# leejet/stable-diffusion.cpp

Hardware: AMD Instinct MI355X
Metric: denoise it/s (image-iterations/s: cond+uncond UNet forwards per image per step) (higher is better)
Workload: dtype f16; 1 GPU; sd15 UNet 512x512, cfg 7 (cond+uncond), f16 weights, batch 8/GPU, Euler-A step; global_batch=8, flash_attn=True, hip_graph=1, cfg_pair_in_one_graph=True, device_resident_sampler=True

## Files before the change

include/ggml-mi355x.h:

```cpp
#ifndef GGML_MI355X_H
#define GGML_MI355X_H

#include "ggml-abi.h"

#ifdef __cplusplus
extern "C" {
#endif

#define GGML_MI355X_API __attribute__((visibility("default")))

GGML_MI355X_API ggml_backend_reg_t ggml_backend_init(void);
GGML_MI355X_API int ggml_backend_score(void);
GGML_MI355X_API ggml_backend_reg_t ggml_backend_mi355x_reg(void);
GGML_MI355X_API int ggml_backend_mi355x_get_device_count(void);

struct ggml_backend_mi355x_stats {
    int64_t graphs_computed;
    int64_t plans_built;
    int64_t nodes_seen;
    int64_t kernels_planned;
    int64_t kernels_launched;
    int64_t fused_conv;
    int64_t fused_conv_bounced;
    int64_t fused_linear;
// ... 16 lines not shown
    int64_t fused_proj_tokens;
    int64_t gemm_attention;
    int64_t fused_q16;
    int64_t split_k_inlaunch;
    int64_t qgemm16_linears;
    int64_t fgemv_linears;
    int64_t fused_presilu;
    int64_t fused_sibling_linears;
    int64_t hoisted_kv_linears;
    int64_t window_convs;
    int64_t hoisted_emb_linears;
    int64_t fused_rows16;
    int64_t fused_joint_qkv;
    int64_t jit_images;
    int64_t fused_cat_rows16;
    int64_t fused_gn_stats;
    int64_t fused_ln_reduce;
    int64_t redirect_fallbacks;
    int64_t fused_concat_gn;
    int64_t fused_conv_scale;
    int64_t view_graphs;
    int64_t plans_evicted;
    int64_t hoisted_mod_linears;
    int64_t view_external_nodes;
    int64_t qinloop_linears;
    int64_t flash_out_alias;
    int64_t flash_slice_images;
    int64_t flash_short_launches;
    int64_t flash_qb2_launches;
    int64_t flash_mslot_launches;
    int64_t flash_generic_launches;
    int64_t fused_gn_epilogue;
    int64_t fused_tile_merge;
};
GGML_MI355X_API void ggml_backend_mi355x_get_stats(struct ggml_backend_mi355x_stats* out);
GGML_MI355X_API int ggml_backend_mi355x_resolve_enums(const char* (*op_name)(int), const char* (*unary_op_name)(int), const char* (*type_name)(int));
GGML_MI355X_API const char* ggml_backend_mi355x_enum_status(void);
GGML_MI355X_API void ggml_backend_mi355x_get_enum_maps(uint8_t* ops256, uint8_t* unary256);
struct ggml_backend_mi355x_kernel_timing {
    char kernel[96];
    int64_t launches;
    double total_ms;
    double total_flops;
    double total_bytes;
    int32_t bound;
    int32_t family;
};
GGML_MI355X_API void ggml_backend_mi355x_kernel_timing_enable(int enable);
GGML_MI355X_API void ggml_backend_mi355x_kernel_timing_enable_mask(uint32_t family_mask);
GGML_MI355X_API void ggml_backend_mi355x_get_kernel_timing(struct ggml_backend_mi355x_kernel_timing* out);
GGML_MI355X_API int ggml_backend_mi355x_get_kernel_timings(struct ggml_backend_mi355x_kernel_timing* out, int capacity);
GGML_MI355X_API void ggml_backend_mi355x_set_option(const char* key, int value);
struct ggml_backend_mi355x_calibration {
    float mfma_f16_tflops;
    float mfma_clock_mhz;
    float copy_tbs;
    float read_tbs;
    int compute_units;
};
GGML_MI355X_API int ggml_backend_mi355x_calibrate(struct ggml_backend_mi355x_calibration* out);
GGML_MI355X_API void* ggml_backend_mi355x_get_stream(ggml_backend_t backend);
GGML_MI355X_API bool ggml_backend_mi355x_step_cache_probe(ggml_backend_t backend, const float* x, float c_in, const float* prev_in, int64_t n, float* stats);
GGML_MI355X_API bool ggml_backend_mi355x_step_cache_record(ggml_backend_t backend, const float* in, const float* out, float* prev_in, float* prev_out, float* diff, int64_t per,
                                                           int k, int64_t nb, bool has_prev_out, float* stats);
GGML_MI355X_API bool ggml_backend_mi355x_step_cache_probe_rel(ggml_backend_t backend, const float* x, float c_in, const float* prev_in, int64_t n, float* stats);
GGML_MI355X_API bool ggml_backend_mi355x_spectrum_predict(ggml_backend_t backend, const float* ring, int64_t slot_stride, const int* order, int k, const float* weights, float w,
                                                          int64_t n, float* out);
GGML_MI355X_API bool ggml_backend_mi355x_spectrum_push(ggml_backend_t backend, const float* src, float* dst, int64_t n);
GGML_MI355X_API const char* ggml_backend_mi355x_hip_library(void);
GGML_MI355X_API int ggml_backend_mi355x_set_device(int hip_device);
GGML_MI355X_API int ggml_backend_mi355x_get_device(void);

#ifdef __cplusplus
}
#endif
#endif
```

stable-diffusion.cpp_amd/__init__.py:

```python
from __future__ import annotations

import ctypes as C
import os
from pathlib import Path

import numpy as np

PKG_DIR = Path(__file__).resolve().parent
ROOT = PKG_DIR.parent
LIB_DIR = PKG_DIR / "lib"
HOST_LIB = Path(os.environ.get("SDCPP_HOST_LIB", str(LIB_DIR / "libsdcpp-host.so")))
BACKEND_LIB = Path(os.environ.get("SDCPP_BACKEND_LIB", str(LIB_DIR / "libggml-mi355x.so")))

F32, F16, Q4_0, Q8_0, I32, BF16 = 0, 1, 2, 8, 26, 30
TYPE_SIZE = {F32: 4, F16: 2, BF16: 2, I32: 4}

SD15, SDXL, SD15_TINY, SDXL_TINY, SD35_LARGE, SD35_TINY, FLUX_DEV, FLUX_TINY, SD35_WIDE2, FLUX_WIDE1, SD3M_TINY, SD35_WIDE8, FLUX_WIDE8 = 0, 1, 2, 3, 4, 5, 6, 7, 8, 9, 10, 11, 12
PAIR_EXCHANGE_FN = C.CFUNCTYPE(C.c_bool, C.c_void_p, C.c_int64, C.c_void_p, C.c_void_p)
EVAL_CALLBACK_FN = C.CFUNCTYPE(C.c_bool, C.c_void_p, C.c_bool, C.c_void_p)
EULER, EULER_A, HEUN, DPM2, DPMPP2S_A, DPMPP2M, DPMPP2Mv2, IPNDM, IPNDM_V, LCM, DDIM_TRAILING = range(11)
TCD, RES_MULTISTEP, RES_2S, ER_SDE, EULER_CFG_PP, EULER_A_CFG_PP, EULER_GE, DPMPP2M_SDE, DPMPP2M_SDE_BT, LMS = range(11, 21)
SAMPLE_METHOD_DEFAULT = 21
SCHED_DISCRETE, SCHED_KARRAS, SCHED_EXPONENTIAL, SCHED_AYS, SCHED_GITS, SCHED_SGM_UNIFORM, SCHED_SIMPLE, SCHED_SMOOTHSTEP, SCHED_KL_OPTIMAL, SCHED_LCM = range(10)
SCHED_BONG_TANGENT, SCHED_FLUX, SCHED_BETA, SCHEDULER_DEFAULT = 10, 14, 15, 16
# ... 319 lines not shown
    L.sd_get_learned_condition.restype = C.c_bool
    L.sdm_set_backend_eval_callback.argtypes = [EVAL_CALLBACK_FN, C.c_void_p]
    L.sdm_set_backend_eval_callback.restype = None
    L.sdm_backend_graph_compute_with_eval_callback.argtypes = [C.c_void_p, C.c_void_p, EVAL_CALLBACK_FN, C.c_void_p]
    L.sdm_backend_graph_compute_with_eval_callback.restype = C.c_int
    _lib = L
    return L


_loaded_plugins: set[str] = set()


def load_backend(path: os.PathLike | str) -> None:
    p = str(Path(path).resolve())
    if p in _loaded_plugins:
        return
    if not lib().sd_load_backend(p.encode()):
        raise EngineError(f"failed to load backend plug-in {p}")
    _loaded_plugins.add(p)


def load_mi355x_backend() -> None:
    if not BACKEND_LIB.exists():
        raise EngineError(f"{BACKEND_LIB} missing — the HIP backend was not built")
    load_backend(BACKEND_LIB)
    names = devices()
    if not any(n.upper().startswith("MI355X") for n in names):
        raise EngineError(f"libggml-mi355x.so loaded but exposes no MI355X device (devices: {names}); is a gfx950 GPU visible?")


_BACKEND_STAT_FIELDS = ("graphs_computed plans_built nodes_seen kernels_planned kernels_launched fused_conv fused_conv_bounced fused_linear "
                        "fused_norm fused_geglu fused_attention generic_matmul swizzled_weight_bytes graph_replays fused_linear_geglu "
                        "split_k_gemms head_major_gemms fused_modulate fused_gate fused_gelu fused_rope fused_concat_heads qgemv_linears fused_chan_add fused_proj_tokens gemm_attention fused_q16 split_k_inlaunch qgemm16_linears fgemv_linears fused_presilu fused_sibling_linears hoisted_kv_linears window_convs hoisted_emb_linears fused_rows16 fused_joint_qkv jit_images fused_cat_rows16 fused_gn_stats fused_ln_reduce redirect_fallbacks fused_concat_gn fused_conv_scale view_graphs plans_evicted hoisted_mod_linears view_external_nodes qinloop_linears flash_out_alias flash_slice_images "
                        "flash_short_launches flash_qb2_launches flash_mslot_launches flash_generic_launches fused_gn_epilogue fused_tile_merge").split()


class BackendStats(C.Structure):
    _fields_ = [(n, C.c_int64) for n in _BACKEND_STAT_FIELDS]


_backend_cdll = None


def _backend() -> C.CDLL:
    global _backend_cdll
    if _backend_cdll is None:
        load_mi355x_backend()
        _backend_cdll = C.CDLL(str(BACKEND_LIB))
        _backend_cdll.ggml_backend_mi355x_get_stats.argtypes = [C.POINTER(BackendStats)]
        _backend_cdll.ggml_backend_mi355x_set_option.argtypes = [C.c_char_p, C.c_int]
    return _backend_cdll


def backend_stats() -> dict:
    st = BackendStats()
    _backend().ggml_backend_mi355x_get_stats(C.byref(st))
    return {n: int(getattr(st, n)) for n in _BACKEND_STAT_FIELDS}


class KernelTiming(C.Structure):
    _fields_ = [("kernel", C.c_char * 96), ("launches", C.c_int64), ("total_ms", C.c_double), ("total_flops", C.c_double),
                ("total_bytes", C.c_double), ("bound", C.c_int32), ("family", C.c_int32)]


KF_ALL = 0x3FFFF


# ... 722 lines not shown
```

stable-diffusion.cpp_amd/csrc/backend/backend.cpp:

```cpp
#include <hip/hip_runtime.h>

#include <atomic>
#include <cstdio>
#include <cstdlib>
#include <cstring>
#include <mutex>
#include <string>
#include <vector>

#include "ggml-abi.h"
#include "ggml-abi-check.h"
#include <dlfcn.h>
#include <link.h>

#include "ggml-mi355x.h"
#include "ktime.h"
#include "planner.h"
#include "kernels.h"

namespace mi355x {

#define HIP_OK(expr)                                                                                          \
    do {                                                                                                      \
        hipError_t _e = (expr);                                                                               \
// ... 364 lines not shown
    return (int)mi355x::g_devices.size();
}
GGML_MI355X_API void ggml_backend_mi355x_get_stats(struct ggml_backend_mi355x_stats* out) { mi355x::planner_get_stats(out); }
GGML_MI355X_API int ggml_backend_mi355x_calibrate(struct ggml_backend_mi355x_calibration* out) {
    mi355x::CalibrationResult r;
    if (!out || !mi355x::calibrate_device(nullptr, &r)) return -1;
    out->mfma_f16_tflops = r.mfma_f16_tflops;
    out->mfma_clock_mhz  = r.mfma_clock_mhz;
    out->copy_tbs        = r.copy_tbs;
    out->read_tbs        = r.read_tbs;
    out->compute_units   = r.compute_units;
    return 0;
}
GGML_MI355X_API int ggml_backend_mi355x_resolve_enums(const char* (*op_name)(int), const char* (*unary_op_name)(int), const char* (*type_name)(int)) {
    std::lock_guard<std::mutex> lk(mi355x::g_enum_mu);
    const bool was_ok = mi355x::g_enum_ok;
    const std::string was = mi355x::g_enum_status;
    const bool ok = mi355x::resolve_host_enums(op_name, unary_op_name, type_name, "ggml_backend_mi355x_resolve_enums");
    if (ok) {
        mi355x::g_enum_explicit = true;
    } else {
        mi355x::g_enum_ok     = was_ok;
        mi355x::g_enum_status = mi355x::g_enum_status + " [previous state kept: " + was + "]";
    }
    return ok ? 0 : -1;
}
GGML_MI355X_API const char* ggml_backend_mi355x_enum_status(void) {
    std::lock_guard<std::mutex> lk(mi355x::g_enum_mu);
    static thread_local std::string copy;
    copy = mi355x::g_enum_status;
    return copy.c_str();
}
GGML_MI355X_API void ggml_backend_mi355x_get_enum_maps(uint8_t* ops256, uint8_t* unary256) { mi355x::planner_get_op_maps(ops256, unary256); }
GGML_MI355X_API void ggml_backend_mi355x_set_option(const char* key, int value) {
    if (strcmp(key, "pinned_uploads") == 0) {
        mi355x::g_pinned_uploads.store(value);
        return;
    }
    mi355x::planner_set_option(key, value);
}
static void fill_timing(struct ggml_backend_mi355x_kernel_timing* o, const mi355x::KFamTiming& t, int family) {
    memset(o, 0, sizeof(*o));
    snprintf(o->kernel, sizeof(o->kernel), "%s", t.name);
    o->launches    = t.launches;
    o->total_ms    = t.total_ms;
    o->total_flops = t.total_flops;
    o->total_bytes = t.total_bytes;
    o->bound       = t.bound;
    o->family      = family;
}
GGML_MI355X_API void ggml_backend_mi355x_kernel_timing_enable(int enable) { mi355x::ktime_enable(enable ? 1u : 0u); }
GGML_MI355X_API void ggml_backend_mi355x_kernel_timing_enable_mask(uint32_t family_mask) { mi355x::ktime_enable(family_mask); }
GGML_MI355X_API void* ggml_backend_mi355x_get_stream(ggml_backend_t backend) {
    return backend ? (void*)((mi355x::BackendCtx*)backend->context)->stream : nullptr;
}
static float* step_cache_scratch(mi355x::BackendCtx* c) {
    if (!c->step_cache_partial && hipMalloc((void**)&c->step_cache_partial, mi355x::step_cache_partial_bytes()) != hipSuccess) {
        (void)hipGetLastError();
        c->step_cache_partial = nullptr;
    }
    return c->step_cache_partial;
}
GGML_MI355X_API bool ggml_backend_mi355x_step_cache_probe(ggml_backend_t backend, const float* x, float c_in, const float* prev_in, int64_t n, float* stats) {
    if (!backend || !x || !prev_in || !stats) return false;
    mi355x::BackendCtx* c = (mi355x::BackendCtx*)backend->context;
    if (hipSetDevice(c->dev->id) != hipSuccess) return false;
// ... 64 lines not shown
```

stable-diffusion.cpp_amd/csrc/backend/planner.cpp:

```cpp
#include "planner.h"

#include <atomic>
#include <cstddef>
#include <cstdio>
#include <cstdlib>
#include <cstring>
#include <functional>
#include <memory>
#include <mutex>
#include <string>
#include <algorithm>
#include <map>
#include <unordered_map>
#include <unordered_set>
#include <vector>

#include "kernels.h"
#include "ktime.h"

namespace mi355x {

static uint8_t g_opmap[256];
static uint8_t g_unmap[256];
static bool g_opmap_init = [] {
// ... 76 lines not shown
        err_len = sizeof(local);
    }
    static const char* const kOptionalOps[]   = {"CONV_2D"};
    static const char* const kOptionalUnary[] = {"EXP"};
    if (op_name && !build_map(op_name, kNeededOps, (int)(sizeof(kNeededOps) / sizeof(kNeededOps[0])), 200, GGML_OP_COUNT, ops, err, err_len, "op", kOptionalOps, 1)) return false;
    if (unary_name && !build_map(unary_name, kNeededUnary, (int)(sizeof(kNeededUnary) / sizeof(kNeededUnary[0])), 64, GGML_UNARY_OP_COUNT, un, err, err_len, "unary op", kOptionalUnary, 1))
        return false;
    if (type_name) {
        for (const NameNum& t : kNeededTypes) {
            const char* nm = type_name(t.num);
            if (!nm || strcmp(nm, t.name)) {
                snprintf(err, err_len, "host ggml_type %d is named '%s', this backend was written against '%s'", t.num, nm ? nm : "(null)", t.name);
                return false;
            }
        }
    }
    if (op_name) memcpy(g_opmap, ops, 256);
    if (unary_name) memcpy(g_unmap, un, 256);
    return true;
}
void planner_get_op_maps(uint8_t* ops256, uint8_t* unary256) {
    if (ops256) memcpy(ops256, g_opmap, 256);
    if (unary256) memcpy(unary256, g_unmap, 256);
}

namespace {

constexpr size_t N_STATS = sizeof(ggml_backend_mi355x_stats) / sizeof(int64_t);
static_assert(N_STATS * sizeof(int64_t) == sizeof(ggml_backend_mi355x_stats), "ggml_backend_mi355x_stats: int64_t fields only");
std::atomic<int64_t> g_stat_counters[N_STATS];
#define STAT(field) g_stat_counters[offsetof(ggml_backend_mi355x_stats, field) / sizeof(int64_t)]

struct Options {
    std::atomic<int> fusion{1}, mfma_gemm{1}, hip_graph{1}, flash_pattern{1}, fuse_modulate{1}, fuse_gate{1}, fuse_gelu{1}, fuse_rope{1}, fuse_concat_heads{1}, qgemv{1}, fuse_chan_add{1}, fuse_proj_tokens{1}, fuse_q16{1}, qgemm16{1}, fgemv{1}, fuse_siblings{1}, hoist_kv{1}, hoist_emb{1}, fuse_rows16{0}, fuse_cat_rows16{1}, fuse_joint_qkv{1}, jit_qimages{4096}, fuse_gn_stats{1}, fuse_ln_reduce{1}, relax_res_overlap{1}, fuse_split_gelu{1}, fuse_concat_gn{1}, fuse_gn_tokens{1}, fuse_linear_nchw{1}, fuse_conv_scale{1}, ignore_use_counts{0}, plan_cache_cap{512}, hoist_mod{1}, fuse_flash_slices{1}, fuse_act_pack{1}, fuse_gn_epilogue{1}, fuse_tile_merge{1};
} g_opt;

using Step = std::function<void(hipStream_t)>;

struct Plan {
    int n_nodes = 0;
    uint64_t check = 0;
    size_t arena_needed = 0;
    std::vector<Step> steps;
    hipGraphExec_t graph_exec = nullptr;
    bool graph_failed         = false;
    int64_t runs              = 0;
    uint64_t last_use         = 0;
};

struct SwzEntry {
    void* swz;
    size_t bytes;
    const void* src;
    size_t src_bytes;
};

std::mutex g_mu;
std::vector<Planner*> g_planners;

}

struct Planner {
    int device;
    std::mutex mu;
    uint64_t tick = 0;
    std::unordered_map<uint64_t, std::unique_ptr<Plan>> plans;
    std::unordered_map<uint64_t, SwzEntry> swz;
// ... 830 lines not shown
        return;
    }
    if (g_opt.fgemv && plain_epi && simple_rows && src_safe && emit_node == i && fgemv_supported((int)w->type, tokens, K) && aligned16(w->data)) {
        float* fdst       = (float*)gi.node(last)->data;
        const float* fx   = (const float*)xsrc->data;
        const int64_t fxs = (int64_t)x->nb[1] / 4;
        const void* wp    = w->data;
        const int wt      = (int)w->type;
        const bool silu   = xsrc != x;
        B.emit([=](hipStream_t st) { launch_fgemv(st, fdst, M, fx, fxs, tokens, wp, wt, K, M, ep, silu); });
        STAT(fgemv_linears)++;
        STAT(fused_linear)++;
        if (silu) STAT(fused_presilu)++;
        return;
    }
    if (xsrc != x) {
        float* ud       = (float*)x->data;
        const float* us = (const float*)xsrc->data;
        const int64_t un = ggml_abi_nelements(x);
        B.emit([=](hipStream_t st) { launch_unary(st, UN_SILU, ud, us, un); });
    }
    const bool useq  = g_opt.qgemm16 && hm_d == 0 && geglu_out < 0 && qgemm16_supported((int)w->type, tokens, K, M);
    const void* wraw = w->data;
    const int wt     = (int)w->type;
    const bool qin = !useq && geglu_out < 0 && hm_d == 0 && !B.hm_hoisting && nchw_add < 0 && (wt == 8 || wt == 2) &&
                     (int64_t)w->nb[1] == (int64_t)ggml_abi_row_size(w->type, K) && aligned16(w->data) && gemm16_qinloop_supported(wt, tokens, M, K, 1, 1);
    if (qin) {
        ep.qtype      = wt;
        ep.qrow_bytes = (int64_t)w->nb[1];
        STAT(qinloop_linears)++;
    }
    const bool jit = !useq && !qin && g_opt.jit_qimages > 0 && tokens >= g_opt.jit_qimages && geglu_out < 0 && hm_d == 0 && !B.hm_hoisting && wswz_q_supported((int)w->type, K) &&
                     (int64_t)w->nb[1] == (int64_t)ggml_abi_row_size(w->type, K) && aligned16(w->data);
    const int geglu_mode = geglu_out >= 0 ? gemm16_geglu_mode(tokens, M, K) : 0;
    const void* swz = useq ? nullptr : qin ? w->data : (jit ? B.P->jit_buffer(wswz_bytes(M, K), B.jit_seq[wswz_bytes(M, K)]++) : get_swz_linear(B.P, w, s, geglu_mode));
    if (jit && swz) {
        void* jb          = const_cast<void*>(swz);
        const void* wsrc  = w->data;
        const int wty     = (int)w->type;
        B.emit_at(emit_node, i, [=](hipStream_t st) { launch_wswz_q(st, jb, wsrc, wty, K, M); });
        STAT(jit_images)++;
    }
    float* dst      = (float*)gi.node(last)->data;
    const float* xp = (const float*)x->data;
    const int64_t xs = (int64_t)x->nb[1] / 4;
    const ggml_tensor* key = strip_reshape(x);
    auto it = B.packed.find(key);
    if (it == B.packed.end() || it->second.nhwc) {
        Packed pk{B.alloc((size_t)tokens * rup64(K) * 2), rup64(K), false};
        Planner* P = B.P;
        const size_t off = pk.off;
        const bool runs  = x->ne[2] > 1 && x->nb[2] != x->nb[1] * (size_t)x->ne[1];
        const int64_t pL = runs ? x->ne[1] : 0, pbs = runs ? (int64_t)x->nb[2] / 4 : 0;
        B.emit([=](hipStream_t st) { launch_pack_rows_f16(st, P->arena + off, xp, tokens, K, xs, pL, pbs); });
        it = B.packed.emplace(key, pk).first;
        if (it->second.nhwc) it->second = pk;
    }
    Planner* P       = B.P;
    size_t off       = it->second.off;
    const int64_t ld = it->second.ld;
    if (it->second.runL > 0) {
        const int64_t rL = it->second.runL, rS = it->second.runS;
        if (geglu_out >= 0 || hm_d > 0 || nchw_add >= 0) {
            const size_t goff = B.alloc((size_t)tokens * ld * 2), soff = off;
            const int64_t nrun = tokens / rL;
            B.emit([=](hipStream_t st) {
                for (int64_t r = 0; r < nrun; ++r)
                    (void)hipMemcpyAsync(P->arena + goff + (size_t)(r * rL * ld * 2), P->arena + soff + (size_t)(r * rS * ld * 2), (size_t)(rL * ld * 2), hipMemcpyDeviceToDevice, st);
            });
            off = goff;
        } else {
            ep.a_run_L = rL;
            ep.a_run_S = rS;
        }
    }
    if (nchw_add >= 0 && !useq && swz && ld == rup64(K) && geglu_out < 0 && gelu_out < 0 && !ep.gate && !redir) {
        float* ndst             = (float*)gi.node(nchw_add)->data;
        const int64_t HWt = nchw_HW, Nimg = nchw_N;
        const float* resp       = nchw_res;
        const Builder::Split sk = B.plan_split(tokens, M, rup64(K), true, true);
        const bool rec_want = g_opt.fuse_gn_epilogue && feeds_group_norm(gi, nchw_add);
        const bool rec_on  = sk.S <= 1 && rec_want && gemm16_conv_gn_rec_supported(HWt, Nimg, M, rup64(K), 1);
        const size_t rec_o = rec_on ? B.alloc((size_t)Nimg * (HWt / GN_REC_CHUNK) * M * sizeof(GnRec)) : 0;
        if (rec_on) B.gn_rec[gi.node(nchw_add)] = rec_o;
        B.emit_at(emit_node, i, [=](hipStream_t st) {
            Epilogue e2 = ep;
            e2.residual = resp;
            if (rec_on) e2.gn_rec = (GnRec*)(P->arena + rec_o);
            launch_gemm16_conv(st, ndst, P->arena + off, swz, HWt, 1, K, Nimg, M, 1, 1, 0, false, e2, sk.ws(P), sk.cnt(P), sk.S);
        });
        STAT(fused_linear)++;
        STAT(fused_proj_tokens)++;
        return;
    }
    if (nchw_add >= 0) {
        while (!chain.empty() && chain.back() != last) chain.pop_back();
    }
    if (geglu_out >= 0) {
        const size_t ooff  = B.alloc((size_t)tokens * (M / 2) * 2);
        const float* biasp = ep.bias;
        const Builder::Split sk = B.plan_split(tokens, M, K, false, false, true);
        B.emit([=](hipStream_t st) { launch_gemm16_linear_geglu(st, P->arena + ooff, P->arena + off, ld, swz, tokens, K, M, biasp, sk.ws(P), sk.cnt(P), sk.S, geglu_mode); });
        B.packed[gi.node(geglu_out)] = Packed{ooff, M / 2, false};
        STAT(fused_geglu)++;
        STAT(fused_linear_geglu)++;
    } else if (gelu_out >= 0) {
        const size_t ooff = B.alloc((size_t)tokens * M * 2);
        if (useq) {
            B.emit([=](hipStream_t st) { launch_qgemm16(st, nullptr, P->arena + ooff, M, P->arena + off, ld, tokens, wraw, wt, K, M, ep); });
            STAT(qgemm16_linears)++;
        } else {
            const Builder::Split sk = B.plan_split(tokens, M, K, false, false);
            B.emit([=](hipStream_t st) { launch_gemm16_linear(st, nullptr, P->arena + ooff, M, P->arena + off, ld, swz, tokens, K, M, M, ep, 0, 0, 0, sk.ws(P), sk.cnt(P), sk.S); });
        }
        B.packed[gi.node(gelu_out)] = Packed{ooff, M, false};
        STAT(fused_gelu)++;
    } else if (hm_d > 0) {
        void* hdst = gi.node(last)->data;
        STAT(head_major_gemms)++;
        const bool f16o = hm_f16;
        const int hd = hm_d, hH = hm_H, hL = hm_L;
        int qflash = -1, qview = -1;
        if (!f16o && g_opt.fuse_q16 && hd % 8 == 0) {
            const int c1 = gi.sole(last);
            const int c2 = (c1 >= 0 && xop(gi.node(c1)) == GGML_OP_RESHAPE) ? gi.sole(c1) : -1;
            if (c2 >= 0 && xop(gi.node(c2)) == GGML_OP_FLASH_ATTN_EXT && gi.node(c2)->src[0] == gi.node(c1) && !gi.node(c2)->src[3] && contig(gi.node(c1)) &&
                gi.node(c1)->ne[0] == hd && flash_attn_supported(hd, gi.node(c2)->src[2]->ne[0])) {
                qflash = c2;
                qview  = c1;
            }
        }
        const bool groupable = B.hm_grouping && !ep.residual && !ep.gate && !ep.gelu && !ep.chan_add;
        if (qflash >= 0) {
            const size_t qoff        = B.alloc((size_t)tokens * M * 2);
            B.q16[gi.node(qview)]    = qoff;
// ... 82 lines not shown
                    if (b2 < 0 || b2 % 4 != 0 || col2 + v2->ne[0] > c0) others_ok = false;
                }
                if (!others_ok) continue;
                split_on  = true;
                split_c0  = c0;
                split_ld  = cp->second.ld;
                split_off = cp->second.off + (size_t)cp->second.col * 2;
                B.cat16[cp->second.cat].written[cp->second.part] = true;
                B.cat16_by_linear.insert(gi.node(jc));
                STAT(fused_gelu)++;
                break;
            }
        }
        B.emit_at(emit_node, i, [=](hipStream_t st) {
            Epilogue e2 = ep;
            if (split_on) {
                e2.split_col   = split_c0;
                e2.split_dst16 = P->arena + split_off;
                e2.split_ldd16 = split_ld;
            }
            if (ln_on) {
                e2.ln_dst16 = P->arena + ln_off;
                e2.ln_w     = lnw;
                e2.ln_b     = lnb;
                e2.ln_eps   = lneps;
            }
            launch_gemm16_linear(st, redir ? (float*)(P->arena + redir_off) : dst, nullptr, 0, P->arena + off, ld, swz, tokens, K, M, M, e2, 0, 0, 0, sk.ws(P), sk.cnt(P), sk.S);
        });
        if (redir) B.redirect_taken.insert(gi.node(last));
    }
    STAT(fused_linear)++;
}

static Step hm_single_step(Planner* P, const Builder::HmLaunch& h) {
    return [=](hipStream_t st) {
        launch_gemm16_linear(st, h.dst, h.dst16_arena ? (void*)(P->arena + h.dst16_off) : h.dst16, 0, P->arena + h.a_off, h.lda, h.swz, h.tokens, h.K, h.M, h.M, h.ep, h.hd, h.hH, h.hL);
    };
}

static bool read_only_after(const GInfo& gi, int k, int pos, const std::vector<int>& members) {
    for (int c : gi.consumers[k]) {
        bool in = false;
        for (int m : members) in = in || m == c;
        if (in) continue;
        if (ggml_abi_op_is_noop(xop(gi.node(c)))) {
            if (!read_only_after(gi, c, pos, members)) return false;
        } else if (c <= pos) {
            return false;
        }
    }
    return true;
}

void plan_sibling_group(Builder& B, int i, hipStream_t s, std::vector<int>& chain) {
    GInfo& gi            = B.gi;
    Planner* P           = B.P;
    const ggml_tensor* n = gi.node(i);
    const ggml_tensor* x = n->src[1];
    const ggml_tensor* w = n->src[0];
    std::vector<int> members = chain;
    int emit_pos = i;
    for (int c : chain) emit_pos = std::max(emit_pos, c);
    if (g_opt.fuse_siblings) {
        std::vector<int> sib;
        for (int c = i + 1; c < gi.g->n_nodes && c < i + 64; ++c) {
            const ggml_tensor* m = gi.node(c);
            if (!gi.done[c] && xop(m) == GGML_OP_MUL_MAT && m->src[1] == x && m->src[0] != w && linear_fast_ok(m) && m->src[0]->type == w->type && m->src[0]->ne[0] == w->ne[0] &&
// ... 4 lines not shown
            if (B.hm_group.size() >= 4) break;
            std::vector<int> cj;
            B.emit_redirect = j;
            plan_linear(B, j, s, cj);
            B.emit_redirect = -1;
            for (int c : cj) {
                gi.done[c] = 1;
                members.push_back(c);
            }
        }
    }
    B.hm_grouping = false;
    const Builder::HmLaunch& h0 = B.hm_group[0];
    bool fuse = B.hm_group.size() >= 2;
    for (const auto& h : B.hm_group) {
        fuse = fuse && h.a_off == h0.a_off && h.lda == h0.lda && h.tokens == h0.tokens && h.K == h0.K && h.M == h0.M && h.hd == h0.hd && h.hH == h0.hH && h.hL == h0.hL &&
               h.ep.scale == h0.ep.scale;
        emit_pos = std::max(emit_pos, h.out_node);
    }
    for (const auto& h : B.hm_group) fuse = fuse && read_only_after(gi, h.out_node, emit_pos, members);
    if (!fuse) {
        for (const auto& h : B.hm_group) {
            if (h.node == i)
                B.emit(hm_single_step(P, h));
            else
                B.deferred[h.node].push_back(hm_single_step(P, h));
        }
        B.hm_group.clear();
        return;
    }
    const std::vector<Builder::HmLaunch> grp = B.hm_group;
    B.hm_group.clear();
    STAT(fused_sibling_linears) += (int64_t)grp.size() - 1;
    B.emit_at(emit_pos, i, [=](hipStream_t st) {
        float* dst[16]        = {};
        void* dst16[16]       = {};
        const void* wswz[16]  = {};
        const float* bias[16] = {};
        const int nn = (int)grp.size();
        for (int k = 0; k < nn; ++k) {
            dst[k]   = grp[k].dst;
            dst16[k] = grp[k].dst16_arena ? (void*)(P->arena + grp[k].dst16_off) : grp[k].dst16;
            wswz[k]  = grp[k].swz;
            bias[k]  = grp[k].ep.bias;
        }
        launch_gemm16_linear_multi(st, nn, dst, dst16, P->arena + grp[0].a_off, grp[0].lda, wswz, grp[0].tokens, grp[0].K, grp[0].M, bias, grp[0].ep.scale, grp[0].hd, grp[0].hH,
                                   grp[0].hL);
    });
}

void plan_hoisted_kv(Builder& B, hipStream_t s) {
    if (!g_opt.hoist_kv || !g_opt.fusion || !g_opt.fuse_siblings) return;
    GInfo& gi  = B.gi;
    Planner* P = B.P;
    struct Key {
        const ggml_tensor* x;
        int wtype;
        int64_t K, M, d, H, L;
        bool operator<(const Key& o) const { return std::tie(x, wtype, K, M, d, H, L) < std::tie(o.x, o.wtype, o.K, o.M, o.d, o.H, o.L); }
    };
    std::map<Key, std::vector<int>> groups;
    for (int j = 0; j < gi.g->n_nodes; ++j) {
        const ggml_tensor* n = gi.node(j);
        if (xop(n) != GGML_OP_MUL_MAT || !linear_fast_ok(n)) continue;
        const ggml_tensor* x  = n->src[1];
        const ggml_tensor* xr = strip_reshape(x);
        if (!(gi.idx(xr) < 0 || xop(xr) == GGML_OP_REPEAT)) continue;
        const int j1 = gi.sole(j);
        const int j2 = (j1 >= 0 && xop(gi.node(j1)) == GGML_OP_RESHAPE) ? gi.sole(j1) : -1;
        const int j3 = (j2 >= 0 && xop(gi.node(j2)) == GGML_OP_PERMUTE) ? gi.sole(j2) : -1;
        const int j4 = (j3 >= 0 && xop(gi.node(j3)) == GGML_OP_CONT) ? gi.sole(j3) : -1;
        const int j5 = (j4 >= 0 && xop(gi.node(j4)) == GGML_OP_RESHAPE) ? gi.sole(j4) : -1;
        if (j5 < 0 || xop(gi.node(j5)) != GGML_OP_CPY || gi.node(j5)->type != GGML_TYPE_F16) continue;
        int jf = -1, nread = 0;
        for (int c : gi.consumers[j5])
            if (c != j5) {
                jf = c;
// ... 2460 lines not shown

namespace {
struct OptionRow {
    const char* key;
    std::atomic<int> Options::*member;
    void (*setter)(int);
};
#define OPT(name) {#name, &Options::name, nullptr}
const OptionRow g_option_table[] = {
    OPT(fusion),
    OPT(mfma_gemm),
    OPT(hip_graph),
    OPT(flash_pattern),
    {"gemm16_t320", nullptr, gemm16_set_t320},
    {"t256p_pad", nullptr, gemm16_set_t256p_pad},
    {"tail_split", nullptr, gemm16_set_tail_split},
    {"conv_wmajor", nullptr, gemm16_set_conv_wmajor},
    {"ln16_rows", nullptr, gemm16_set_ln16_rows},
    {"t320_linear_max_split", nullptr, gemm16_set_t320_linear_max_split},
    OPT(qgemv),
    OPT(fuse_q16),
    {"streamk", nullptr, gemm16_set_streamk},
    {"geglu16", nullptr, gemm16_set_geglu16},
    {"bn64_max_tiles", nullptr, gemm16_set_bn64_max},
    {"conv3w_prio", nullptr, conv3w_set_prio},
    {"t256p_min_nt_sk", nullptr, gemm16_set_t256p_min_nt_sk},
    {"t256p_min_tiles_sk", nullptr, gemm16_set_t256p_min_tiles_sk},
    {"conv3w", nullptr, conv3w_set},
    OPT(hoist_emb),
    OPT(fuse_rows16),
    OPT(fuse_cat_rows16),
    OPT(fuse_gn_stats),
    OPT(fuse_gn_epilogue),
    OPT(fuse_tile_merge),
    OPT(fuse_joint_qkv),
    OPT(fuse_ln_reduce),
    OPT(jit_qimages),
    {"qinloop_min_rows", nullptr, gemm16_set_qinloop_min_rows},
    OPT(fuse_flash_slices),
    {"gemm16_t192p", nullptr, gemm16_set_t192p},
    {"conv3w_min_blocks", nullptr, conv3w_set_min_blocks},
    {"conv3w_min_blocks_deep", nullptr, conv3w_set_min_blocks_deep},
    {"gemm16_bn64", nullptr, gemm16_set_bn64},
    OPT(qgemm16),
    {"qgemv_max_rows", nullptr, qgemv_set_max_rows},
    OPT(fgemv),
    OPT(fuse_siblings),
    OPT(hoist_kv),
    {"fgemv_max_rows", nullptr, fgemv_set_max_rows},
    {"qgemm16_max_rows", nullptr, qgemm16_set_max_rows},
    {"qgemm16_rb", nullptr, qgemm16_set_rb},
    {"splitk_inkernel", nullptr, gemm16_set_splitk_inkernel},
    {"splitk_in_target", nullptr, gemm16_set_splitk_in_target},
    OPT(fuse_chan_add),
    OPT(fuse_proj_tokens),
    OPT(fuse_modulate),
    OPT(fuse_gate),
    OPT(relax_res_overlap),
    OPT(fuse_split_gelu),
    OPT(fuse_concat_gn),
    OPT(fuse_gn_tokens),
    OPT(fuse_linear_nchw),
    OPT(fuse_conv_scale),
    OPT(fuse_act_pack),
    OPT(hoist_mod),
    OPT(plan_cache_cap),
// ... 39 lines not shown
```

stable-diffusion.cpp_amd/csrc/kernels/kernels.h:

```cpp
#pragma once
#include <hip/hip_runtime.h>
#include <stddef.h>
#include <stdint.h>

namespace mi355x {

struct View4 {
    const void* data;
    int64_t ne[4];
    int64_t nb[4];
    int type;
};

enum BinOp { BIN_ADD = 0, BIN_SUB = 1, BIN_MUL = 2, BIN_DIV = 3 };
enum UnOp { UN_SILU = 0, UN_GELU = 1, UN_GELU_QUICK = 2, UN_SIGMOID = 3, UN_TANH = 4, UN_RELU = 5, UN_NEG = 6, UN_EXP = 7 };

void launch_binary(hipStream_t s, BinOp op, void* dst, const int64_t dnb[4], const View4& a, const View4& b);
constexpr int TILE_MERGE_MAX = 32;
struct TileMergeTile {
    int x, y, w, h;
    int64_t src;
    int64_t wx, wy;
};
struct TileMergeArgs {
// ... 76 lines not shown
    int64_t split_col     = 0;
    void* split_dst16     = nullptr;
    int64_t split_ldd16   = 0;
    int qtype             = 0;
    int64_t qrow_bytes    = 0;
    int64_t a_run_L       = 0;
    int64_t a_run_S       = 0;
};
void gemm16_init();
bool gemm16_qinloop_supported(int wtype, int64_t rows, int64_t M, int64_t K, int mul, int split);
void gemm16_set_qinloop_min_rows(int v);
void gemm16_set_t192p(int v);
void gemm16_set_tap_major(int v);
int gemm16_tap_major();
void gemm16_set_splitk_target(int v);
void gemm16_set_splitk_mid(int v);
void gemm16_set_tile(int t);
#ifdef MI355X_EXPERIMENTS
void gemm16_set_abl(int v);
#endif
void gemm16_set_t320(int v);
void gemm16_set_t256p_pad(int v);
void gemm16_set_conv_wmajor(int v);
void gemm16_set_ln16_rows(int v);
void gemm16_set_tail_split(int v);
void gemm16_set_bn64(int v);
void gemm16_set_variant(int v);
void launch_gemm16_linear(hipStream_t s, float* dst, void* dst16, int64_t ldd16, const void* a16, int64_t lda, const void* wswz, int64_t rows,
                          int64_t K, int64_t M, int64_t ldd, const Epilogue& ep, int hm_d = 0, int hm_H = 0, int hm_L = 0, float* splitk_ws = nullptr, int* splitk_cnt = nullptr, int splitk_S = 0);
void launch_gemm16_linear_multi(hipStream_t s, int n, float* const* dst, void* const* dst16, const void* a16, int64_t lda, const void* const* wswz, int64_t rows,
                               int64_t K, int64_t M, const float* const* bias, float scale, int hm_d, int hm_H, int hm_L);
void launch_gemm16_linear_geglu(hipStream_t s, void* dst16, const void* a16, int64_t lda, const void* wswz_geglu, int64_t rows, int64_t K, int64_t M,
                                const float* bias, float* splitk_ws = nullptr, int* splitk_cnt = nullptr, int splitk_S = 0, int geglu_mode = 1);
int gemm16_geglu_mode(int64_t rows, int64_t M, int64_t K);
void gemm16_set_bn64_max(int v);
void gemm16_set_geglu16(int v);
int gemm16_split_k(int64_t rows, int64_t M, int64_t K, bool conv);
bool splitk_reduce_gn_supported(int64_t hw, int64_t C, int64_t N, int groups);
bool splitk_reduce_ln_supported(int64_t rows, int64_t M);
void gemm16_set_t320_linear_max_split(int v);
struct G16SplitPlan {
    int S;
    bool inkernel;
    size_t ws_bytes;
    int tiles;
};
G16SplitPlan gemm16_split_plan(int64_t rows, int64_t M, int64_t K, bool conv, bool plain_out, bool geglu = false);
void gemm16_set_splitk_inkernel(int v);
void gemm16_set_splitk_in_target(int v);
void launch_gemm16_conv(hipStream_t s, float* dst, const void* x16_nhwc, const void* wswz, int64_t W, int64_t H, int64_t IC, int64_t N, int64_t OC,
                        int ksize, int stride, int pad, bool upscale2x, const Epilogue& ep, float* splitk_ws = nullptr, int* splitk_cnt = nullptr, int splitk_S = 0);
bool gemm16_conv_gn_rec_supported(int64_t OHOW, int64_t N, int64_t OC, int64_t ICp, int ksize);
int conv3w_plan(int64_t W, int64_t H, int64_t IC, int64_t N, int64_t OC, int ksize, int stride, bool upscale2x, int* bn_out = nullptr);
void launch_conv3w(hipStream_t s, float* dst, const void* x16_nhwc, const void* wswz32, int64_t W, int64_t H, int64_t IC, int64_t N, int64_t OC, const Epilogue& ep,
                   float* splitk_ws, int S);
bool conv3w_gn_rec_supported(int64_t OHOW, int64_t OC, int64_t N);
void qgemm16_set_rb(int v);
void conv3w_set_prio(int v);
void conv3w_set(int v);
void conv3w_set_min_blocks(int v);
void conv3w_set_min_blocks_deep(int v);
void launch_pack_rows_f16(hipStream_t s, void* dst, const float* x, int64_t R, int64_t K, int64_t xs, int64_t L = 0, int64_t bs = 0);
void launch_pack_cols_f16(hipStream_t s, void* dst, int64_t ld, const float* x, int64_t R, int64_t K, int64_t xs, bool gelu);
void launch_layer_norm_f16(hipStream_t s, void* dst, const float* x, int64_t ne0, int64_t nrows, int64_t x_stride, float eps, const float* w,
                           const float* b, bool rms, int64_t mod_L = 0);
void launch_geglu_f16(hipStream_t s, void* dst, const float* x, int64_t tokens, int64_t inner, int64_t x_stride);
// ... 58 lines not shown
```

Measured before the change: 376.0 it/s.

## Add row-panel GEMM kernel for K=320/640 head-major and GEGLU linears

Adds a new GEMM kernel that keeps each wave's activation rows (K=320 or 640) resident in registers and streams 32-column weight tiles through double-buffered LDS. A block covers one row panel and a range of column tiles. The planner routes single and sibling head-major QKV/KV linears with plain f16 epilogues, and FF1+GEGLU at K=320, to this kernel by default. The goal is to cut repeated activation reloads and improve MFMA feeding for these small-K projections. The cost is a large register footprint and a separate code path that needs alignment checks.

```diff
diff --git a/include/ggml-mi355x.h b/include/ggml-mi355x.h
--- a/include/ggml-mi355x.h
+++ b/include/ggml-mi355x.h
@@ -72,6 +72,7 @@
     int64_t flash_generic_launches;
     int64_t fused_gn_epilogue;
     int64_t fused_tile_merge;
+    int64_t rowpanel_linears;
 };
 GGML_MI355X_API void ggml_backend_mi355x_get_stats(struct ggml_backend_mi355x_stats* out);
 GGML_MI355X_API int ggml_backend_mi355x_resolve_enums(const char* (*op_name)(int), const char* (*unary_op_name)(int), const char* (*type_name)(int));
@@ -91,6 +92,8 @@
 GGML_MI355X_API void ggml_backend_mi355x_get_kernel_timing(struct ggml_backend_mi355x_kernel_timing* out);
 GGML_MI355X_API int ggml_backend_mi355x_get_kernel_timings(struct ggml_backend_mi355x_kernel_timing* out, int capacity);
 GGML_MI355X_API void ggml_backend_mi355x_set_option(const char* key, int value);
+GGML_MI355X_API int ggml_backend_mi355x_rowpanel_plan(int64_t rows, int64_t K, int64_t M, int n_weights, int f16_out, int plain_epilogue, int hm_d, int hm_L, int geglu_mode, int cus,
+                                                     int* ranges, int* tiles_per_range, int* tile_cols, int* panel_rows);
 struct ggml_backend_mi355x_calibration {
     float mfma_f16_tflops;
     float mfma_clock_mhz;
diff --git a/stable-diffusion.cpp_amd/__init__.py b/stable-diffusion.cpp_amd/__init__.py
--- a/stable-diffusion.cpp_amd/__init__.py
+++ b/stable-diffusion.cpp_amd/__init__.py
@@ -375,7 +375,7 @@
 _BACKEND_STAT_FIELDS = ("graphs_computed plans_built nodes_seen kernels_planned kernels_launched fused_conv fused_conv_bounced fused_linear "
                         "fused_norm fused_geglu fused_attention generic_matmul swizzled_weight_bytes graph_replays fused_linear_geglu "
                         "split_k_gemms head_major_gemms fused_modulate fused_gate fused_gelu fused_rope fused_concat_heads qgemv_linears fused_chan_add fused_proj_tokens gemm_attention fused_q16 split_k_inlaunch qgemm16_linears fgemv_linears fused_presilu fused_sibling_linears hoisted_kv_linears window_convs hoisted_emb_linears fused_rows16 fused_joint_qkv jit_images fused_cat_rows16 fused_gn_stats fused_ln_reduce redirect_fallbacks fused_concat_gn fused_conv_scale view_graphs plans_evicted hoisted_mod_linears view_external_nodes qinloop_linears flash_out_alias flash_slice_images "
-                        "flash_short_launches flash_qb2_launches flash_mslot_launches flash_generic_launches fused_gn_epilogue fused_tile_merge").split()
+                        "flash_short_launches flash_qb2_launches flash_mslot_launches flash_generic_launches fused_gn_epilogue fused_tile_merge rowpanel_linears").split()
 
 
 class BackendStats(C.Structure):
diff --git a/stable-diffusion.cpp_amd/csrc/backend/backend.cpp b/stable-diffusion.cpp_amd/csrc/backend/backend.cpp
--- a/stable-diffusion.cpp_amd/csrc/backend/backend.cpp
+++ b/stable-diffusion.cpp_amd/csrc/backend/backend.cpp
@@ -420,6 +420,15 @@
     return copy.c_str();
 }
 GGML_MI355X_API void ggml_backend_mi355x_get_enum_maps(uint8_t* ops256, uint8_t* unary256) { mi355x::planner_get_op_maps(ops256, unary256); }
+GGML_MI355X_API int ggml_backend_mi355x_rowpanel_plan(int64_t rows, int64_t K, int64_t M, int n_weights, int f16_out, int plain_epilogue, int hm_d, int hm_L, int geglu_mode, int cus,
+                                                     int* ranges, int* tiles_per_range, int* tile_cols, int* panel_rows) {
+    if (cus < 1 || !mi355x::rowpanel_linear_supported(rows, K, M, n_weights, f16_out != 0, plain_epilogue != 0, hm_d, hm_L, geglu_mode)) return 0;
+    const int bn = mi355x::rowpanel_tile_cols(K);
+    if (tile_cols) *tile_cols = bn;
+    if (panel_rows) *panel_rows = mi355x::rowpanel_panel_rows(K);
+    return mi355x::rowpanel_grid(rows, (int64_t)n_weights * ((M + bn - 1) / bn), K, cus, ranges, tiles_per_range);
+}
+
 GGML_MI355X_API void ggml_backend_mi355x_set_option(const char* key, int value) {
     if (strcmp(key, "pinned_uploads") == 0) {
         mi355x::g_pinned_uploads.store(value);
diff --git a/stable-diffusion.cpp_amd/csrc/backend/planner.cpp b/stable-diffusion.cpp_amd/csrc/backend/planner.cpp
--- a/stable-diffusion.cpp_amd/csrc/backend/planner.cpp
+++ b/stable-diffusion.cpp_amd/csrc/backend/planner.cpp
@@ -132,7 +132,7 @@
 #define STAT(field) g_stat_counters[offsetof(ggml_backend_mi355x_stats, field) / sizeof(int64_t)]
 
 struct Options {
-    std::atomic<int> fusion{1}, mfma_gemm{1}, hip_graph{1}, flash_pattern{1}, fuse_modulate{1}, fuse_gate{1}, fuse_gelu{1}, fuse_rope{1}, fuse_concat_heads{1}, qgemv{1}, fuse_chan_add{1}, fuse_proj_tokens{1}, fuse_q16{1}, qgemm16{1}, fgemv{1}, fuse_siblings{1}, hoist_kv{1}, hoist_emb{1}, fuse_rows16{0}, fuse_cat_rows16{1}, fuse_joint_qkv{1}, jit_qimages{4096}, fuse_gn_stats{1}, fuse_ln_reduce{1}, relax_res_overlap{1}, fuse_split_gelu{1}, fuse_concat_gn{1}, fuse_gn_tokens{1}, fuse_linear_nchw{1}, fuse_conv_scale{1}, ignore_use_counts{0}, plan_cache_cap{512}, hoist_mod{1}, fuse_flash_slices{1}, fuse_act_pack{1}, fuse_gn_epilogue{1}, fuse_tile_merge{1};
+    std::atomic<int> fusion{1}, mfma_gemm{1}, hip_graph{1}, flash_pattern{1}, fuse_modulate{1}, fuse_gate{1}, fuse_gelu{1}, fuse_rope{1}, fuse_concat_heads{1}, qgemv{1}, fuse_chan_add{1}, fuse_proj_tokens{1}, fuse_q16{1}, qgemm16{1}, fgemv{1}, fuse_siblings{1}, hoist_kv{1}, hoist_emb{1}, fuse_rows16{0}, fuse_cat_rows16{1}, fuse_joint_qkv{1}, jit_qimages{4096}, fuse_gn_stats{1}, fuse_ln_reduce{1}, relax_res_overlap{1}, fuse_split_gelu{1}, fuse_concat_gn{1}, fuse_gn_tokens{1}, fuse_linear_nchw{1}, fuse_conv_scale{1}, ignore_use_counts{0}, plan_cache_cap{512}, hoist_mod{1}, fuse_flash_slices{1}, fuse_act_pack{1}, fuse_gn_epilogue{1}, fuse_tile_merge{1}, rowpanel_linear{1};
 } g_opt;
 
 using Step = std::function<void(hipStream_t)>;
@@ -1029,7 +1029,10 @@
     }
     const bool jit = !useq && !qin && g_opt.jit_qimages > 0 && tokens >= g_opt.jit_qimages && geglu_out < 0 && hm_d == 0 && !B.hm_hoisting && wswz_q_supported((int)w->type, K) &&
                      (int64_t)w->nb[1] == (int64_t)ggml_abi_row_size(w->type, K) && aligned16(w->data);
-    const int geglu_mode = geglu_out >= 0 ? gemm16_geglu_mode(tokens, M, K) : 0;
+    const auto rp_pk     = B.packed.find(strip_reshape(x));
+    const bool rp_a_ok   = rp_pk == B.packed.end() || rp_pk->second.nhwc || (rp_pk->second.ld % 8 == 0 && (rp_pk->second.runL > 0 || rp_pk->second.off % 16 == 0));
+    const bool rp_geglu  = geglu_out >= 0 && !useq && rp_a_ok && g_opt.rowpanel_linear && (M / 2) % 16 == 0 && rowpanel_linear_supported(tokens, K, M, 1, true, true, 0, 0, 2);
+    const int geglu_mode = geglu_out >= 0 ? (rp_geglu ? 2 : gemm16_geglu_mode(tokens, M, K)) : 0;
     const void* swz = useq ? nullptr : qin ? w->data : (jit ? B.P->jit_buffer(wswz_bytes(M, K), B.jit_seq[wswz_bytes(M, K)]++) : get_swz_linear(B.P, w, s, geglu_mode));
     if (jit && swz) {
         void* jb          = const_cast<void*>(swz);
@@ -1096,8 +1099,21 @@
     if (geglu_out >= 0) {
         const size_t ooff  = B.alloc((size_t)tokens * (M / 2) * 2);
         const float* biasp = ep.bias;
-        const Builder::Split sk = B.plan_split(tokens, M, K, false, false, true);
-        B.emit([=](hipStream_t st) { launch_gemm16_linear_geglu(st, P->arena + ooff, P->arena + off, ld, swz, tokens, K, M, biasp, sk.ws(P), sk.cnt(P), sk.S, geglu_mode); });
+        if (rp_geglu) {
+            if (!swz || ld % 8 != 0 || off % 16 != 0) {
+                fprintf(stderr, "ggml-mi355x: row-panel FF1 + GEGLU planned on an operand image it cannot read (ld %lld, offset %zu)\n", (long long)ld, off);
+                abort();
+            }
+            B.emit([=](hipStream_t st) {
+                void* d       = P->arena + ooff;
+                const void* wi = swz;
+                launch_rowpanel_linear(st, 1, &d, M / 2, P->arena + off, ld, &wi, tokens, K, M, &biasp, 1.f, 0, 0, 0, 2);
+            });
+            STAT(rowpanel_linears)++;
+        } else {
+            const Builder::Split sk = B.plan_split(tokens, M, K, false, false, true);
+            B.emit([=](hipStream_t st) { launch_gemm16_linear_geglu(st, P->arena + ooff, P->arena + off, ld, swz, tokens, K, M, biasp, sk.ws(P), sk.cnt(P), sk.S, geglu_mode); });
+        }
         B.packed[gi.node(geglu_out)] = Packed{ooff, M / 2, false};
         STAT(fused_geglu)++;
         STAT(fused_linear_geglu)++;
@@ -1246,7 +1262,22 @@
     STAT(fused_linear)++;
 }
 
+static bool hm_rowpanel_ok(const Builder::HmLaunch& h, int n) {
+    const bool plain = !h.ep.residual && !h.ep.gate && !h.ep.gelu && !h.ep.chan_add && !h.ep.qtype && h.ep.a_run_L == 0 && h.ep.split_col == 0 && !h.ep.ln_dst16 && h.ep.act < 0;
+    return g_opt.rowpanel_linear && !h.dst && (h.dst16 || h.dst16_arena) && h.swz && h.lda % 8 == 0 && h.a_off % 16 == 0 &&
+           rowpanel_linear_supported(h.tokens, h.K, h.M, n, true, plain, h.hd, h.hL, 0);
+}
+
 static Step hm_single_step(Planner* P, const Builder::HmLaunch& h) {
+    if (hm_rowpanel_ok(h, 1)) {
+        STAT(rowpanel_linears)++;
+        return [=](hipStream_t st) {
+            void* d        = h.dst16_arena ? (void*)(P->arena + h.dst16_off) : h.dst16;
+            const void* wi = h.swz;
+            const float* b = h.ep.bias;
+            launch_rowpanel_linear(st, 1, &d, 0, P->arena + h.a_off, h.lda, &wi, h.tokens, h.K, h.M, &b, h.ep.scale, h.hd, h.hH, h.hL, 0);
+        };
+    }
     return [=](hipStream_t st) {
         launch_gemm16_linear(st, h.dst, h.dst16_arena ? (void*)(P->arena + h.dst16_off) : h.dst16, 0, P->arena + h.a_off, h.lda, h.swz, h.tokens, h.K, h.M, h.M, h.ep, h.hd, h.hH, h.hL);
     };
@@ -1317,6 +1348,9 @@
     const std::vector<Builder::HmLaunch> grp = B.hm_group;
     B.hm_group.clear();
     STAT(fused_sibling_linears) += (int64_t)grp.size() - 1;
+    bool rowpanel = true;
+    for (const auto& h : grp) rowpanel = rowpanel && hm_rowpanel_ok(h, (int)grp.size());
+    if (rowpanel) STAT(rowpanel_linears)++;
     B.emit_at(emit_pos, i, [=](hipStream_t st) {
         float* dst[16]        = {};
         void* dst16[16]       = {};
@@ -1328,6 +1362,10 @@
             dst16[k] = grp[k].dst16_arena ? (void*)(P->arena + grp[k].dst16_off) : grp[k].dst16;
             wswz[k]  = grp[k].swz;
             bias[k]  = grp[k].ep.bias;
+        }
+        if (rowpanel) {
+            launch_rowpanel_linear(st, nn, dst16, 0, P->arena + grp[0].a_off, grp[0].lda, wswz, grp[0].tokens, grp[0].K, grp[0].M, bias, grp[0].ep.scale, grp[0].hd, grp[0].hH, grp[0].hL, 0);
+            return;
         }
         launch_gemm16_linear_multi(st, nn, dst, dst16, P->arena + grp[0].a_off, grp[0].lda, wswz, grp[0].tokens, grp[0].K, grp[0].M, bias, grp[0].ep.scale, grp[0].hd, grp[0].hH,
                                    grp[0].hL);
@@ -3854,6 +3892,7 @@
     OPT(fuse_cat_rows16),
     OPT(fuse_gn_stats),
     OPT(fuse_gn_epilogue),
+    OPT(rowpanel_linear),
     OPT(fuse_tile_merge),
     OPT(fuse_joint_qkv),
     OPT(fuse_ln_reduce),
diff --git a/stable-diffusion.cpp_amd/csrc/kernels/kernels.h b/stable-diffusion.cpp_amd/csrc/kernels/kernels.h
--- a/stable-diffusion.cpp_amd/csrc/kernels/kernels.h
+++ b/stable-diffusion.cpp_amd/csrc/kernels/kernels.h
@@ -132,6 +132,12 @@
                                int64_t K, int64_t M, const float* const* bias, float scale, int hm_d, int hm_H, int hm_L);
 void launch_gemm16_linear_geglu(hipStream_t s, void* dst16, const void* a16, int64_t lda, const void* wswz_geglu, int64_t rows, int64_t K, int64_t M,
                                 const float* bias, float* splitk_ws = nullptr, int* splitk_cnt = nullptr, int splitk_S = 0, int geglu_mode = 1);
+bool rowpanel_linear_supported(int64_t rows, int64_t K, int64_t M, int n_weights, bool f16_out, bool plain_epilogue, int hm_d, int hm_L, int geglu_mode);
+int rowpanel_tile_cols(int64_t K);
+int rowpanel_panel_rows(int64_t K);
+int rowpanel_grid(int64_t rows, int64_t tiles, int64_t K, int cus, int* ranges_out, int* tiles_per_range_out);
+void launch_rowpanel_linear(hipStream_t s, int n, void* const* dst16, int64_t ldd16, const void* a16, int64_t lda, const void* const* wswz, int64_t rows, int64_t K, int64_t M,
+                            const float* const* bias, float scale, int hm_d, int hm_H, int hm_L, int geglu_mode);
 int gemm16_geglu_mode(int64_t rows, int64_t M, int64_t K);
 void gemm16_set_bn64_max(int v);
 void gemm16_set_geglu16(int v);
diff --git a/stable-diffusion.cpp_amd/csrc/kernels/rowpanel.hip b/stable-diffusion.cpp_amd/csrc/kernels/rowpanel.hip
--- /dev/null
+++ b/stable-diffusion.cpp_amd/csrc/kernels/rowpanel.hip
@@ -0,0 +1,223 @@
+#include <cstdio>
+#include <cstdlib>
+#include <type_traits>
+#include <utility>
+#include "device_utils.h"
+#include "kernels.h"
+#include "ktime.h"
+#include "g16_common.h"
+
+namespace mi355x {
+
+namespace {
+constexpr int RP_MAX_W = 4;
+
+static int rp_num_cus() {
+    int dev = 0, cus = 0;
+    if (hipGetDevice(&dev) != hipSuccess || hipDeviceGetAttribute(&cus, hipDeviceAttributeMultiprocessorCount, dev) != hipSuccess || cus <= 0) cus = 256;
+    return cus;
+}
+static bool rp_trace() {
+    static const bool on = getenv("GGML_MI355X_TRACE") != nullptr;
+    return on;
+}
+}
+
+#define RP_RD(DST_, ADDR_, OFF_) asm volatile("ds_read_b128 %0, %1 offset:%2" : "=v"(DST_) : "v"(ADDR_), "n"(OFF_))
+template <int P, int CB, int PD>
+__device__ __forceinline__ void rp_prefetch(half8_t (&bf)[PD][CB], const uint32_t (&bad)[CB]) {
+#pragma unroll
+    for (int cb = 0; cb < CB; ++cb) RP_RD(bf[P][cb], bad[cb], P * 1024);
+    if constexpr (P + 1 < PD) rp_prefetch<P + 1, CB, PD>(bf, bad);
+}
+template <int KS, int KF, int CB, int PD>
+__device__ __forceinline__ void rp_kstep(const half8_t (&af)[KF], half8_t (&bf)[PD][CB], float16_t (&acc)[1][CB], const uint32_t (&bad)[CB]) {
+    constexpr int left = ((KS + PD < KF ? KS + PD : KF) - KS - 1) * CB;
+    asm volatile("s_waitcnt lgkmcnt(%0)" ::"n"(left) : "memory");
+#pragma unroll
+    for (int cb = 0; cb < CB; ++cb) asm volatile("" : "+v"(bf[KS % PD][cb]));
+    __builtin_amdgcn_sched_barrier(0);
+#pragma unroll
+    for (int cb = 0; cb < CB; ++cb) acc[0][cb] = __builtin_amdgcn_mfma_f32_32x32x16_f16(af[KS], bf[KS % PD][cb], acc[0][cb], 0, 0, 0);
+    __builtin_amdgcn_sched_barrier(0);
+    if constexpr (KS + PD < KF) {
+#pragma unroll
+        for (int cb = 0; cb < CB; ++cb) RP_RD(bf[KS % PD][cb], bad[cb], (KS + PD) * 1024);
+    }
+    __builtin_amdgcn_sched_barrier(0);
+    if constexpr (KS + 1 < KF) rp_kstep<KS + 1, KF, CB, PD>(af, bf, acc, bad);
+}
+
+template <int KF, int CB, int NW, int OCC>
+__global__ __launch_bounds__(NW * 64, OCC) void k_gemm16_rowpanel(G16Args g, int ntiles, int tpr, int nranges) {
+    constexpr int BN   = CB * 32;
+    constexpr int BM   = NW * 32;
+    constexpr int NFR  = CB * KF;
+    constexpr int SLOT = NFR * 1024;
+    constexpr int PW   = (NFR + NW - 1) / NW;
+    constexpr int PD   = KF > 20 ? 8 : 4;
+    static_assert(2 * SLOT <= 160 * 1024 && KF * 1024 <= 65536 && (PD - 1) * CB <= 15 && PD <= KF, "LDS budget, ds_read offset field, lgkmcnt range");
+    __shared__ __attribute__((aligned(1024))) char smem[2 * SLOT];
+    const uint32_t lds0 = (uint32_t)(uintptr_t)(__attribute__((address_space(3))) char*)smem;
+
+    const int lane = threadIdx.x & 63;
+    const int wave = __builtin_amdgcn_readfirstlane(threadIdx.x >> 6);
+    int bid      = blockIdx.x;
+    const int nb = gridDim.x;
+    if ((nb & 7) == 0) bid = (bid & 7) * (nb >> 3) + (bid >> 3);
+    const int panel = bid / nranges, range = bid - panel * nranges;
+    const int t0 = range * tpr, t1 = min(ntiles, t0 + tpr);
+    const int64_t row0 = (int64_t)panel * BM;
+
+    int64_t row = row0 + wave * 32 + (lane & 31);
+    if (row >= g.R) row = g.R - 1;
+    const _Float16* ap = g.A + row * g.lda + (lane >> 5) * 8;
+    half8_t af[KF];
+#pragma unroll
+    for (int ks = 0; ks < KF; ++ks) af[ks] = *(const half8_t*)(ap + ks * 16);
+
+#define RP_PICK(A_, wi_) ((wi_) < 2 ? ((wi_) == 0 ? g.A_[0] : g.A_[1]) : ((wi_) == 2 ? g.A_[2] : g.A_[3]))
+    auto stage = [&](int t, int slot) {
+        int ct           = t;
+        const half8_t* W = g.W;
+        if (g.multi > 1) {
+            const int wi = t / g.ncol_tiles;
+            ct           = t - wi * g.ncol_tiles;
+            W            = RP_PICK(Wm, wi);
+        }
+        const half8_t* src = W + (int64_t)ct * (NFR * 64) + wave * 64 + lane;
+        char* dstp         = smem + slot * SLOT + wave * 1024;
+#pragma unroll
+        for (int q = 0; q < PW; ++q)
+            if (q * NW + NW - 1 < NFR || q * NW + wave < NFR) GLDS16(src + q * (NW * 64), dstp + q * (NW * 1024));
+    };
+
+    if (t0 < t1) stage(t0, 0);
+#pragma unroll
+    for (int ks = 0; ks < KF; ++ks) asm volatile("" : "+v"(af[ks]));
+
+    for (int t = t0; t < t1; ++t) {
+        const int slot = (t - t0) & 1;
+        __builtin_amdgcn_s_waitcnt(0x0F70);
+        __syncthreads();
+        if (t + 1 < t1) stage(t + 1, slot ^ 1);
+
+        float16_t acc[1][CB];
+#pragma unroll
+        for (int cb = 0; cb < CB; ++cb) acc[0][cb] = (float16_t){0};
+        uint32_t bad[CB];
+#pragma unroll
+        for (int cb = 0; cb < CB; ++cb) bad[cb] = lds0 + (uint32_t)(slot * SLOT + cb * KF * 1024 + lane * 16);
+        half8_t bf[PD][CB];
+        asm volatile("s_waitcnt lgkmcnt(0)" ::: "memory");
+        rp_prefetch<0, CB, PD>(bf, bad);
+        __builtin_amdgcn_sched_barrier(0);
+        rp_kstep<0, KF, CB, PD>(af, bf, acc, bad);
+
+        int ct = t;
+        if (g.multi > 1) {
+            const int wi = t / g.ncol_tiles;
+            ct           = t - wi * g.ncol_tiles;
+            g.dst16      = RP_PICK(dst16m, wi);
+            g.ep.bias    = RP_PICK(biasm, wi);
+        }
+        const int col0 = ct * BN;
+        int lane_e     = lane;
+        int64_t row0_e = row0;
+        asm volatile("" : "+v"(lane_e));
+        asm volatile("" : "+s"(row0_e), "+s"(g.ldd16), "+s"(g.hm_d));
+        if (KF == 20 && g.geglu_inner > 0) {
+            if constexpr (KF == 20) epi_geglu16<1, CB>(acc, g, row0_e, col0, wave, 0, lane_e);
+        } else {
+            epi_linear<EPI_HM_F16, 1, CB>(acc, g, row0_e, col0, wave, 0, lane_e);
+        }
+    }
+#undef RP_PICK
+}
+
+bool rowpanel_linear_supported(int64_t rows, int64_t K, int64_t M, int n_weights, bool f16_out, bool plain_epilogue, int hm_d, int hm_L, int geglu_mode) {
+    if ((K != 320 && K != 640) || n_weights < 1 || n_weights > RP_MAX_W) return false;
+    if (!f16_out || !plain_epilogue || rows < 1 || rows >= (1ll << 31) || M < 1) return false;
+    if ((hm_d > 0) == (geglu_mode != 0)) return false;
+    if (hm_d > 0 && hm_L < 32) return false;
+    if (geglu_mode != 0 && (n_weights != 1 || M % 64 != 0 || geglu_mode != 2 || K != 320)) return false;
+    return (int64_t)n_weights * ((M + 31) / 32) < (1 << 20);
+}
+int rowpanel_tile_cols(int64_t K) { return 32; }
+int rowpanel_panel_rows(int64_t K) { return K <= 320 ? 256 : 128; }
+
+int rowpanel_grid(int64_t rows, int64_t tiles, int64_t K, int cus, int* ranges_out, int* tiles_per_range_out) {
+    const int64_t bm     = rowpanel_panel_rows(K);
+    const int64_t panels = (rows + bm - 1) / bm;
+    const int64_t target = (int64_t)cus * 2;
+    int64_t nr           = (target + panels - 1) / panels;
+    const int64_t max_nr = tiles / 2 > 1 ? tiles / 2 : 1;
+    if (nr > max_nr) nr = max_nr;
+    if (nr < 1) nr = 1;
+    const int64_t tpr = (tiles + nr - 1) / nr;
+    nr                = (tiles + tpr - 1) / tpr;
+    if (ranges_out) *ranges_out = (int)nr;
+    if (tiles_per_range_out) *tiles_per_range_out = (int)tpr;
+    return (int)(panels * nr);
+}
+
+void launch_rowpanel_linear(hipStream_t s, int n, void* const* dst16, int64_t ldd16, const void* a16, int64_t lda, const void* const* wswz, int64_t rows, int64_t K, int64_t M,
+                            const float* const* bias, float scale, int hm_d, int hm_H, int hm_L, int geglu_mode) {
+    if (!rowpanel_linear_supported(rows, K, M, n, true, true, hm_d, hm_L, geglu_mode) || lda % 8 != 0 || lda < K || ((uintptr_t)a16 & 15) != 0) {
+        fprintf(stderr, "ggml-mi355x: launch_rowpanel_linear called for a launch it does not support (rows %lld K %lld M %lld x%d)\n", (long long)rows, (long long)K, (long long)M, n);
+        abort();
+    }
+    G16Args g{};
+    g.A     = (const _Float16*)a16;
+    g.lda   = lda;
+    g.kfr   = K / 16;
+    g.R     = rows;
+    g.C     = M;
+    g.ldd   = M;
+    g.ldd16 = ldd16;
+    g.hm_d  = hm_d;
+    g.hm_H  = hm_H;
+    g.hm_L  = hm_L;
+    g.ep    = G16Epi{bias[0], nullptr, scale};
+    g.ncol_tiles = (int)((M + rowpanel_tile_cols(K) - 1) / rowpanel_tile_cols(K));
+    g.multi = n > 1 ? n : 0;
+    for (int i = 0; i < n; ++i) {
+        if (!wswz[i] || !dst16[i]) {
+            fprintf(stderr, "ggml-mi355x: launch_rowpanel_linear needs a resident f16 weight image and an f16 destination per weight\n");
+            abort();
+        }
+        g.Wm[i]     = (const half8_t*)wswz[i];
+        g.dst16m[i] = (_Float16*)dst16[i];
+        g.biasm[i]  = bias[i];
+    }
+    g.W     = g.Wm[0];
+    g.dst16 = g.dst16m[0];
+    const int64_t Kp = K;
+    double flops, bytes;
+    if (geglu_mode) {
+        g.geglu_inner = (int)(M / 2);
+        g.geglu16     = geglu_mode == 2 ? 1 : 0;
+        g.ldd16       = M / 2;
+        flops         = 2.0 * rows * K * M;
+        bytes         = (double)rows * Kp * 2.0 + (double)Kp * ((M + 127) / 128 * 128) * 2.0 + (double)rows * (M / 2) * 2.0;
+        if (rp_trace()) fprintf(stderr, "G16 linear rows=%lld K=%lld M=%lld res=0 hm=0 f16out=1 geglu=1\n", (long long)rows, (long long)K, (long long)M);
+    } else if (n > 1) {
+        flops = 2.0 * n * rows * K * M;
+        bytes = (double)rows * Kp * 2.0 + (double)n * Kp * ((M + 127) / 128 * 128) * 2.0 + (double)n * rows * M * 2.0;
+        if (rp_trace()) fprintf(stderr, "G16 linear x%d rows=%lld K=%lld M=%lld hm=%d\n", n, (long long)rows, (long long)K, (long long)M, hm_d);
+    } else {
+        flops = 2.0 * rows * K * M;
+        bytes = (double)rows * Kp * 2.0 + (double)Kp * ((M + 127) / 128 * 128) * 2.0 + (double)rows * M * 2.0;
+        if (rp_trace()) fprintf(stderr, "G16 linear rows=%lld K=%lld M=%lld res=0 hm=%d f16out=1\n", (long long)rows, (long long)K, (long long)M, hm_d);
+    }
+    const int tiles = n * g.ncol_tiles;
+    int nr = 1, tpr = tiles;
+    const int grid = rowpanel_grid(rows, tiles, K, rp_num_cus(), &nr, &tpr);
+    KScope ks_(s, KF_LINEAR, flops, bytes);
+    if (K == 320)
+        k_gemm16_rowpanel<20, 1, 8, 4><<<dim3((unsigned)grid), dim3(512), 0, s>>>(g, tiles, tpr, nr);
+    else
+        k_gemm16_rowpanel<40, 1, 4, 2><<<dim3((unsigned)grid), dim3(256), 0, s>>>(g, tiles, tpr, nr);
+}
+
+}
```

New measurement: 377.8 it/s, median of 6. No clear change (+0.5%).
